# r9y9/deepvoice3_pytorch

Measured on AMD Instinct MI355X. Metric: mel-frames/sec/node (train step, deepvoice3_ljspeech), higher is better.
Workload: dtype f16x3

## Files before the change

### deepvoice3_pytorch_amd/csrc/api.hip

```cpp
#include "common.h"
#include <atomic>
#include <mutex>
#include <vector>
#include <string.h>

static thread_local char g_err[512] = "";

void dv3_set_error(const char* fmt, ...) {
  va_list ap;
  va_start(ap, fmt);
  vsnprintf(g_err, sizeof(g_err), fmt, ap);
  va_end(ap);
}

int g_dv3_last_conv = 0, g_dv3_last_wgrad = 0;

__device__ uint32_t g_dv3_range_events;
uint32_t* dv3_range_ctr() {
  static uint32_t* ptr = nullptr;
  static std::once_flag once;
  std::call_once(once, [] {
    void* p = nullptr;
    if (hipGetSymbolAddress(&p, HIP_SYMBOL(g_dv3_range_events)) == hipSuccess) ptr = (uint32_t*)p;
  });
// ... 50 lines not shown
  return DV3_OK;
}
extern "C" int dv3_graph_side_end(void* side_stream, void** exec_out, int32_t* n_nodes_out) {
  DV3_REQUIRE(side_stream && exec_out, "graph_side_end: null argument");
  hipGraph_t graph = nullptr;
  hipError_t e = hipStreamEndCapture((hipStream_t)side_stream, &graph);
  if (e != hipSuccess || !graph) {
    dv3_set_error("graph_side_end: hipStreamEndCapture: %s", hipGetErrorString(e));
    return DV3_ELAUNCH;
  }
  size_t n = 0;
  (void)hipGraphGetNodes(graph, nullptr, &n);
  if (n_nodes_out) *n_nodes_out = (int32_t)n;
  *exec_out = nullptr;
  if (n == 0) {
    (void)hipGraphDestroy(graph);
    return DV3_OK;
  }
  hipGraphExec_t exec = nullptr;
  e = hipGraphInstantiate(&exec, graph, nullptr, nullptr, 0);
  (void)hipGraphDestroy(graph);
  if (e != hipSuccess) {
    dv3_set_error("graph_side_end: hipGraphInstantiate: %s", hipGetErrorString(e));
    return DV3_ELAUNCH;
  }
  *exec_out = (void*)exec;
  return DV3_OK;
}
namespace {
__global__ void flag_signal_kernel(unsigned long long* flag, unsigned long long* epoch, int j, int bump) {
  unsigned long long e = *epoch;
  if (bump) {
    e += 1;
    *epoch = e;
  }
  __hip_atomic_store(flag, e * 4096ull + (unsigned long long)j, __ATOMIC_RELEASE, __HIP_MEMORY_SCOPE_AGENT);
}
__global__ void flag_wait_kernel(const unsigned long long* flag, unsigned long long* epoch, int j, int bump, unsigned* err,
                                 long long timeout_ticks) {
  unsigned long long e = *epoch;
  if (bump) {
    e += 1;
    *epoch = e;
  }
  const unsigned long long want = e * 4096ull + (unsigned long long)j;
  const long long t0 = (long long)wall_clock64();
  while (__hip_atomic_load(flag, __ATOMIC_ACQUIRE, __HIP_MEMORY_SCOPE_AGENT) < want) {
    __builtin_amdgcn_s_sleep(16);
    if ((long long)wall_clock64() - t0 > timeout_ticks) {
      atomicAdd(err, 1u);
      break;
    }
  }
}
}
extern "C" int dv3_flag_signal(uint64_t* flag, uint64_t* epoch, int32_t j, int32_t bump, void* stream) {
  DV3_REQUIRE(flag && epoch && j > 0 && j < 4096, "flag_signal: bad arguments");
  hipLaunchKernelGGL(flag_signal_kernel, dim3(1), dim3(1), 0, (hipStream_t)stream, (unsigned long long*)flag,
                     (unsigned long long*)epoch, (int)j, (int)bump);
  return dv3_check_launch("flag_signal");
}
extern "C" int dv3_flag_wait(const uint64_t* flag, uint64_t* epoch, int32_t j, int32_t bump, uint32_t* err,
                             int32_t timeout_ms, void* stream) {
  DV3_REQUIRE(flag && epoch && err && j > 0 && j < 4096 && timeout_ms > 0, "flag_wait: bad arguments");
  hipLaunchKernelGGL(flag_wait_kernel, dim3(1), dim3(1), 0, (hipStream_t)stream, (const unsigned long long*)flag,
                     (unsigned long long*)epoch, (int)j, (int)bump, (unsigned*)err, (long long)timeout_ms * 100000ll);
  return dv3_check_launch("flag_wait");
}
extern "C" int dv3_graph_launch(void* exec, void* stream) {
  DV3_REQUIRE(exec, "graph_launch: null graph");
  hipError_t e = hipGraphLaunch((hipGraphExec_t)exec, (hipStream_t)stream);
  if (e != hipSuccess) {
    dv3_set_error("graph_launch: %s", hipGetErrorString(e));
    return DV3_ELAUNCH;
  }
  return DV3_OK;
}
extern "C" int dv3_graph_destroy(void* exec) {
  if (exec) (void)hipGraphExecDestroy((hipGraphExec_t)exec);
  return DV3_OK;
}

int dv3_conv_census_count();
extern "C" int dv3_debug_get(int what) {
  if (what == 10) return g_dv3_last_conv;
  if (what == 40) return dv3_conv_census_count();
  if (what == 11) return g_dv3_last_wgrad;
  return 0;
}

extern int g_x3_pingpong, g_x3_rel2, g_x3_pp2, g_x3_prio, g_x3_wide, g_x3_pp2_sk_units, g_x3_j1_flat, g_x3_rel8;
extern int g_x3_ks, g_x3_ks_max_blocks, g_x3_ks_min_steps;
extern int g_pp2_ord_u, g_pp2_ord_m, g_pp2_sk, g_pp2_sk_overhead, g_pp2_sk_gain, g_pp2_fast_tail;
extern int g_planes_tile;
extern int g_c8pp_min_tiles, g_c8pp_rf, g_c8pp_nw4, g_c8pp_stagger, g_c8pp_stagger_mask;
extern int g_wgrad_tile, g_wgrad_prio, g_wgrad_taps2_default, g_wgrad_t2_window, g_wgrad_t2_il;
extern int g_wgrad_c8_pf2, g_wgrad_c8_il, g_wgrad_c8_tr;
extern int g_spk_prefetch;
extern int g_gate_c8_fast, g_gate_vec;
extern int g_loss_fast_log;
extern int g_wn_bwd_vec4;
int dv3_conv_census_set(int on);
extern "C" int dv3_debug_set(int what, int value) {
  if (what == 40) return dv3_conv_census_set(value);
  if (what == 29 || what == 31) {
    DV3_REQUIRE(value == 0 || value == 17 || value == 81, "debug_set(%d, %d): LOAD-phase order 0, 17 or 81", what, value);
    (what == 29 ? g_pp2_ord_u : g_pp2_ord_m) = value;
    return DV3_OK;
  }
  DV3_REQUIRE(what != 52 || (value >= 0 && value <= 4), "debug_set(52, %d): wgrad_c8 form 0..4", value);
  static const struct {
    int what;
    int* var;
  } kSwitches[] = {
      {2, &g_wgrad_tile},        {3, &g_x3_pingpong},         {4, &g_planes_tile},      {9, &g_x3_rel2},
      {12, &g_x3_pp2},           {14, &g_x3_prio},            {15, &g_wgrad_prio},      {17, &g_wgrad_taps2_default},
      {18, &g_x3_wide},          {19, &g_c8pp_min_tiles},     {20, &g_wgrad_c8_pf2},    {22, &g_pp2_sk},
      {23, &g_pp2_sk_overhead},  {24, &g_pp2_sk_gain},        {25, &g_x3_pp2_sk_units}, {27, &g_x3_j1_flat},
      {30, &g_c8pp_rf},          {34, &g_c8pp_nw4},           {35, &g_c8pp_stagger},    {36, &g_c8pp_stagger_mask},
      {42, &g_x3_rel8},          {44, &g_x3_ks},              {45, &g_x3_ks_max_blocks}, {46, &g_x3_ks_min_steps},
      {47, &g_wgrad_t2_window},  {48, &g_wgrad_t2_il},        {49, &g_wgrad_c8_il},     {50, &g_pp2_fast_tail},
      {51, &g_wn_bwd_vec4},      {52, &g_wgrad_c8_tr},        {54, &g_spk_prefetch},    {55, &g_gate_vec},
      {56, &g_gate_c8_fast},     {57, &g_loss_fast_log},
  };
  for (const auto& sw : kSwitches)
    if (sw.what == what) {
      *sw.var = value;
      return DV3_OK;
    }
  dv3_set_error("debug_set(%d, %d): no such switch", what, value);
  return DV3_EINVAL;
}

int dv3_decode_read_stamps(void* dst, int64_t bytes);
int dv3_conv_census_read(int what, void* dst, int64_t bytes);
extern "C" int dv3_debug_read(int what, void* dst, int64_t bytes) {
  if (what == 40 || what == 41) return dv3_conv_census_read(what, dst, bytes);
  if (what == 3 && dst) return dv3_decode_read_stamps(dst, bytes);
  dv3_set_error("debug_read(%d): no such buffer", what);
  return DV3_EINVAL;
}

extern "C" const char* dv3_last_error(void) { return g_err; }
extern "C" int dv3_abi_version(void) { return DV3_ABI_VERSION; }

extern "C" int dv3_device_info(int dev, char* name, int name_len, int* n_cu) {
  hipDeviceProp_t prop;
  hipError_t e = hipGetDeviceProperties(&prop, dev);
  if (e != hipSuccess) {
    dv3_set_error("hipGetDeviceProperties: %s", hipGetErrorString(e));
    return DV3_ELAUNCH;
  }
  if (name && name_len > 0) {
    strncpy(name, prop.gcnArchName, (size_t)name_len - 1);
    name[name_len - 1] = 0;
  }
  if (n_cu) *n_cu = prop.multiProcessorCount;
  return DV3_OK;
}

extern "C" int dv3_sizeof(const char* name) {
#define DV3_SZ(T) if (!strcmp(name, #T)) return (int)sizeof(T)
  DV3_SZ(dv3_conv_desc);
  DV3_SZ(dv3_wgrad_desc);
  DV3_SZ(dv3_wn_desc);
  DV3_SZ(dv3_wn_bwd_desc);
  DV3_SZ(dv3_gate_bwd_desc);
  DV3_SZ(dv3_softmax_desc);
  DV3_SZ(dv3_softmax_bwd_desc);
  DV3_SZ(dv3_spec_loss_desc);
  DV3_SZ(dv3_spec_items_desc);
  DV3_SZ(dv3_wn_multi_entry);
  DV3_SZ(dv3_conv_step_desc);
  DV3_SZ(dv3_attn_step_desc);
  DV3_SZ(dv3_decode_entry);
  DV3_SZ(dv3_decode_program);
  DV3_SZ(dv3_attn_fwd_desc);
  DV3_SZ(dv3_spk_layer);
  DV3_SZ(dv3_spk_desc);
  DV3_SZ(dv3_dropout_site);
#undef DV3_SZ
  return -1;
}
```

### deepvoice3_pytorch_amd/csrc/wgrad_gemm_bf16x3.hip

```cpp
#include "common.h"
#include <type_traits>

typedef __bf16 bf16x8 __attribute__((ext_vector_type(8)));
typedef __bf16 bf16x2 __attribute__((ext_vector_type(2)));
typedef float f32x2 __attribute__((ext_vector_type(2)));
typedef float f32x4u __attribute__((ext_vector_type(4), aligned(4)));

namespace {

struct WgradArgs {
  dv3_wgrad_desc d;
  int m_tiles, c_tiles;
  int prio = 0;
};

constexpr int BKT = 32;
constexpr int KB = 4;
constexpr int PAD = 2;

__device__ __forceinline__ void split8(const float (&v)[8], bf16x8& hi, bf16x8& lo) {
#pragma unroll
  for (int i = 0; i < 8; i += 2) {
    const f32x2 f = {v[i], v[i + 1]};
    const bf16x2 h = __builtin_convertvector(f, bf16x2);
// ... 350 lines not shown
    }
  };

  f32x16 acc[JT][2];
#pragma unroll
  for (int j = 0; j < JT; ++j)
#pragma unroll
    for (int a = 0; a < 2; ++a)
#pragma unroll
      for (int r = 0; r < 16; ++r) acc[j][a][r] = 0.f;

  auto mfma_step = [&](int cur) {
    const bf16x8* GsH = smem + cur * BUF;
    const bf16x8* GsL = GsH + KB * LDM;
#pragma unroll
    for (int ks = 0; ks < 2; ++ks) {
      const int k8 = 2 * ks + lhi;
      const int ai = k8 * LDM + wm * 64 + l31;
      const bf16x8 ah0 = GsH[ai], ah1 = GsH[ai + 32];
      bf16x8 al0 = ah0, al1 = ah1;
      if (TERMS == 3) { al0 = GsL[ai]; al1 = GsL[ai + 32]; }
#pragma unroll
      for (int j = 0; j < JT; ++j) {
        const bf16x8* XsH = GsH + GBUF + j * XTAP;
        const int xi = k8 * LDN + wc * 32 + l31;
        const bf16x8 bh = XsH[xi];
        if (TERMS == 1) {
          acc[j][0] = __builtin_amdgcn_mfma_f32_32x32x16_bf16(ah0, bh, acc[j][0], 0, 0, 0);
          acc[j][1] = __builtin_amdgcn_mfma_f32_32x32x16_bf16(ah1, bh, acc[j][1], 0, 0, 0);
          continue;
        }
        const bf16x8 bl = XsH[KB * LDN + xi];
        acc[j][0] = __builtin_amdgcn_mfma_f32_32x32x16_bf16(al0, bh, acc[j][0], 0, 0, 0);
        acc[j][1] = __builtin_amdgcn_mfma_f32_32x32x16_bf16(al1, bh, acc[j][1], 0, 0, 0);
        acc[j][0] = __builtin_amdgcn_mfma_f32_32x32x16_bf16(ah0, bl, acc[j][0], 0, 0, 0);
        acc[j][1] = __builtin_amdgcn_mfma_f32_32x32x16_bf16(ah1, bl, acc[j][1], 0, 0, 0);
        acc[j][0] = __builtin_amdgcn_mfma_f32_32x32x16_bf16(ah0, bh, acc[j][0], 0, 0, 0);
        acc[j][1] = __builtin_amdgcn_mfma_f32_32x32x16_bf16(ah1, bh, acc[j][1], 0, 0, 0);
      }
    }
  };
  using S0 = std::integral_constant<int, 0>;

  if (nsteps > 0) {
    load_step(0, S0{});
    write_step(0, S0{});
  }
  __syncthreads();
  const int prio = args.prio;
  for (int step = 0; step < nsteps; ++step) {
    if (prio == 1) __builtin_amdgcn_s_setprio(3);
    if (step + 1 < nsteps) load_step(step + 1, S0{});
    if (prio == 1) __builtin_amdgcn_s_setprio(0);
    if (prio == 2) __builtin_amdgcn_s_setprio(3);
    mfma_step(step & 1);
    if (prio == 2) __builtin_amdgcn_s_setprio(0);
    if (prio == 1) __builtin_amdgcn_s_setprio(3);
    if (step + 1 < nsteps) write_step((step + 1) & 1, S0{});
    if (prio == 1) __builtin_amdgcn_s_setprio(0);
    __syncthreads();
  }

  const float oscale = MASK ? p.drop_scale : 1.0f;
  const int c = c0 + wc * 32 + l31;
  if (c < Cin) {
#pragma unroll
    for (int j = 0; j < JT; ++j) {
      float* __restrict__ ob = p.out + (int64_t)s * p.out_ss + (int64_t)j * M * p.ldo;
#pragma unroll
      for (int mi = 0; mi < 2; ++mi)
#pragma unroll
        for (int r = 0; r < 16; ++r) {
          const int m = m0 + wm * 64 + mi * 32 + (r & 3) + 8 * (r >> 2) + 4 * lhi;
          if (m < M) ob[(int64_t)m * p.ldo + c] = acc[j][mi][r] * oscale;
        }
    }
  }
}

}

int g_wgrad_taps2_default = 1;
int dv3_wgrad_taps2_dispatch(const dv3_wgrad_desc* d, hipStream_t st);
int g_wgrad_taps_default = 1;
int g_wgrad_prio = 0;
int g_wgrad_tile = 0;

template <bool MASK, int TERMS>
static int launch_wgrad_taps_t(const WgradArgs& a, int64_t nb, hipStream_t st) {
  constexpr int LDM = 128 + PAD;
  constexpr size_t lds = (size_t)2 * (2 * KB * LDM + 3 * 2 * KB * LDM) * 16;
  static bool attr_set = false;
  if (!attr_set) {
    hipError_t e = hipFuncSetAttribute((const void*)wgrad_taps_kernel<MASK, TERMS>,
                                       hipFuncAttributeMaxDynamicSharedMemorySize, 160 * 1024);
    if (e != hipSuccess) {
      dv3_set_error("wgrad_taps: hipFuncSetAttribute: %s", hipGetErrorString(e));
      return DV3_ELAUNCH;
    }
    attr_set = true;
  }
  hipLaunchKernelGGL((wgrad_taps_kernel<MASK, TERMS>), dim3((unsigned)nb), dim3(512), lds, st, a);
  return dv3_check_launch("wgrad_taps");
}
static int launch_wgrad_taps(const WgradArgs& a, int64_t nb, hipStream_t st) {
  const dv3_wgrad_desc* d = &a.d;
  if (d->split_bf16 == 2)
    return d->xmask ? launch_wgrad_taps_t<true, 1>(a, nb, st) : launch_wgrad_taps_t<false, 1>(a, nb, st);
  return d->xmask ? launch_wgrad_taps_t<true, 3>(a, nb, st) : launch_wgrad_taps_t<false, 3>(a, nb, st);
}

template <int WM, int WN>
static int launch_wgrad_x3(const WgradArgs& a, int64_t nb, hipStream_t st) {
  const dv3_wgrad_desc* d = &a.d;
  dim3 grid((unsigned)nb), block(WM * WN * 64);
  if (d->split_bf16 == 2) {
    if (d->xmask) {
      hipLaunchKernelGGL((wgrad_gemm_bf16x3_kernel<WM, WN, true, 1>), grid, block, 0, st, a);
    } else {
      hipLaunchKernelGGL((wgrad_gemm_bf16x3_kernel<WM, WN, false, 1>), grid, block, 0, st, a);
    }
  } else if (d->xmask) {
    hipLaunchKernelGGL((wgrad_gemm_bf16x3_kernel<WM, WN, true, 3>), grid, block, 0, st, a);
  } else {
    hipLaunchKernelGGL((wgrad_gemm_bf16x3_kernel<WM, WN, false, 3>), grid, block, 0, st, a);
  }
  return dv3_check_launch("wgrad_gemm_bf16x3");
}

int dv3_wgrad_gemm_bf16x3_dispatch(const dv3_wgrad_desc* d, hipStream_t st) {
  if ((int64_t)d->B * d->g_bs + (int64_t)d->M * d->g_rs >= (1ll << 30) ||
      (int64_t)d->B * d->x_bs + (int64_t)d->Cin * d->x_rs >= (1ll << 30) ||
      (d->xmask && (int64_t)d->B * d->Cin * d->xmask_rs >= (1ll << 30)))
    return 1;
  WgradArgs a;
  a.d = *d;
  a.prio = g_wgrad_prio;
  if (d->J == 3 && d->k_split && d->split_bf16 != 2 && (g_wgrad_tile == 4 || (g_wgrad_tile == 0 && g_wgrad_taps2_default)) &&
      (int64_t)(d->B - 1) * d->g_bs + (int64_t)(d->M - 1) * d->g_rs + d->T >= 8 &&
      (int64_t)(d->B - 1) * d->x_bs + (int64_t)(d->Cin - 1) * d->x_rs + d->Tin >= 8)
    return dv3_wgrad_taps2_dispatch(d, st);
  if (d->J == 3 && d->k_split && (g_wgrad_tile == 3 || (g_wgrad_tile == 0 && g_wgrad_taps_default))) {
    a.m_tiles = dv3_cdiv(d->M, 128);
    a.c_tiles = dv3_cdiv(d->Cin, 128);
    const int64_t nb = (int64_t)a.m_tiles * a.c_tiles * d->n_slabs;
    DV3_REQUIRE(nb < (1ll << 31), "wgrad_gemm: grid too large");
    g_dv3_last_wgrad = (d->split_bf16 == 2 ? 4000 : 3000) + 30;
    return launch_wgrad_taps(a, nb, st);
  }
  const bool big = g_wgrad_tile == 2;
  const int bm = big ? 256 : 128;
  a.m_tiles = dv3_cdiv(d->M, bm);
  a.c_tiles = dv3_cdiv(d->Cin, 128);
  const int64_t nb = (int64_t)a.m_tiles * a.c_tiles * d->J * d->n_slabs;
  DV3_REQUIRE(nb < (1ll << 31), "wgrad_gemm: grid too large");
  g_dv3_last_wgrad = (d->split_bf16 == 2 ? 4000 : 3000) + (big ? 20 : 10);
  return big ? launch_wgrad_x3<4, 2>(a, nb, st) : launch_wgrad_x3<2, 2>(a, nb, st);
}
```

### deepvoice3_pytorch_amd/ops.py

```python
import contextlib
import ctypes
import functools
import math

import torch

from . import _lib
from ._lib import CONSTS, STRUCTS, _env_flag, _env_int, _env_str

EPI_LINEAR = CONSTS["DV3_EPI_LINEAR"]
EPI_RELU = CONSTS["DV3_EPI_RELU"]
EPI_SIGMOID = CONSTS["DV3_EPI_SIGMOID"]
EPI_GLU = CONSTS["DV3_EPI_GLU"]
EPI_HIGHWAY = CONSTS["DV3_EPI_HIGHWAY"]
EPI_DGRAD = CONSTS["DV3_EPI_DGRAD"]
EPI_SOFTSIGN = CONSTS["DV3_EPI_SOFTSIGN"]
STORE_BCT = CONSTS["DV3_STORE_BCT"]
STORE_INTERLEAVE2 = CONSTS["DV3_STORE_INTERLEAVE2"]

_conv_desc = STRUCTS["dv3_conv_desc"]
_wgrad_desc = STRUCTS["dv3_wgrad_desc"]
_wn_desc = STRUCTS["dv3_wn_desc"]
_wn_bwd_desc = STRUCTS["dv3_wn_bwd_desc"]
_gate_bwd_desc = STRUCTS["dv3_gate_bwd_desc"]
# ... 831 lines not shown
    return dv, dg, dbias


class WnBwdBatch(object):
    active = False
    group = CONSTS["DV3_WN_BWD_MULTI_MAX"]
    _q, _keep, _dv = [], [], set()

    @classmethod
    def add(cls, d, rows, keep):
        if d.dv in cls._dv:
            cls.flush()
        c = type(d)()
        ctypes.memmove(ctypes.byref(c), ctypes.byref(d), ctypes.sizeof(d))
        cls._q.append(c)
        cls._keep.append(keep)
        cls._dv.add(d.dv)
        if len(cls._q) >= cls.group:
            cls.flush()

    @classmethod
    def flush(cls):
        if not cls._q:
            return
        q, keep = cls._q, cls._keep
        cls._q, cls._keep, cls._dv = [], [], set()
        arr = (type(q[0]) * len(q))(*q)
        _lib.call("dv3_weight_norm_bwd_multi", ctypes.byref(arr), len(q), _stream())
        if SideStream.stream is not None:
            SideStream.retain(keep)

    @classmethod
    def discard(cls):
        cls._q, cls._keep, cls._dv = [], [], set()


def transpose(x, add=None, alpha=1.0):
    x = _c(_chk(x, "x"))
    B, R, C = x.shape
    y = torch.empty((B, C, R), dtype=torch.float32, device=x.device)
    _lib.call("dv3_transpose_f32", x.data_ptr(), y.data_ptr(), _ptr(add), B, R, C, float(alpha), _stream())
    return y


def axpby(a, b, alpha):
    a = _c(a)
    out = torch.empty_like(a)
    _lib.call("dv3_axpby_f32", a.data_ptr(), _ptr(_c(b) if b is not None else None), out.data_ptr(),
              a.numel(), float(alpha), _stream())
    return out


def _ksplit_count(total_steps, tiles, slots=512, min_steps=None, c8=False):
    if min_steps is None:
        min_steps = max(8, min(28, total_steps // 12)) if c8 else max(8, min(32, total_steps // 14))
    return _ksplit_count_c(total_steps, tiles, slots, min_steps)


@functools.lru_cache(maxsize=None)
def _ksplit_count_c(total_steps, tiles, slots, min_steps):
    s_max = max(1, total_steps // min_steps)
    if tiles >= slots:
        return 1
    best, best_eff = 1, 0.0
    for s in range(1, min(s_max, slots) + 1):
        blocks = tiles * s
        rounds = -(-blocks // slots)
        eff = blocks / float(rounds * slots)
        eff *= 1.0 - 0.008 * s
        if eff > best_eff:
            best, best_eff = s, eff
    return best


@functools.lru_cache(maxsize=None)
def _slab_count(B, tiles):
    want = max(1, (512 + tiles - 1) // tiles)
    s = min(B, want)
    while B % s:
        s -= 1
    return max(s, 1)


def wgrad_plan(B, Mg, Cin, Tg, Jd):
    tiles = ((Mg + 127) // 128) * ((Cin + 127) // 128) * Jd
    x3 = _gemm_mode != "f32" and not (Mg <= 64 and Cin <= 64)
    if x3 and Jd == 3:
        S = _ksplit_count(B * ((Tg + 31) // 32), tiles // 3, slots=256)
    elif x3:
        S = _ksplit_count(B * ((Tg + 31) // 32), tiles)
    else:
        S = _slab_count(B, tiles)
    return x3, S


class LayerCfg(object):
    __slots__ = ("k", "dil", "causal", "mode", "residual", "p", "training", "transposed", "site",
                 "pad_left", "t_out", "out_c8")

    def __init__(self, k=1, dil=1, causal=False, mode=EPI_LINEAR, residual=False, p=0.0,
                 training=False, transposed=False, site=None, pad_left=None, t_out=None, out_c8=None):
        self.k, self.dil, self.causal, self.mode = k, dil, causal, mode
        self.residual, self.p, self.training, self.transposed, self.site = residual, p, training, transposed, site
        self.pad_left, self.t_out = pad_left, t_out
        self.out_c8 = out_c8


def _pad_left(k, dil, causal):
    return (k - 1) * dil if causal else (k - 1) // 2 * dil


slab_rows_default = _env_flag("DV3_SLAB_ROWS", True)

grad_ready_hooks = []


class SideStream(object):
    stream = None
    main = None
    keep = []
    capturing = False
    split_capture = False
    split_on_fork = None
    release_every = 4
    _n = 0
    _events = []

    class _Section(object):

        def __enter__(self):
            _stream_override.handle = SideStream.stream.cuda_stream

        def __exit__(self, *exc):
            _stream_override.handle = None
            SideStream._release_point()
            return False

    forks_last = 0
    forks = 0

    @classmethod
    def fork(cls, *tensors):
        cls.forks += 1
        if cls.split_capture:
            if cls.split_on_fork is not None:
                cls.split_on_fork()
        else:
            _lib.call("dv3_stream_fork", cls.main.cuda_stream, cls.stream.cuda_stream)
        cls.keep.append([None, [tensors]])
        return cls._section

    @classmethod
    def retain(cls, *tensors):
        if cls.keep:
            cls.keep[-1][1].append(tensors)
        else:
            cls.keep.append([None, [tensors]])

    @classmethod
    def _release_point(cls):
        cls._n += 1
        if cls.capturing or cls.stream is None or cls._n % cls.release_every:
            return
        done = -1
        for i, (ev, _) in enumerate(cls.keep):
            if ev is not None:
                if not ev.query():
                    break
                done = i
        if done >= 0:
# ... 181 lines not shown
            ctx.has_bias = bias is not None
            ctx.save_for_backward(x, v, g, ab if gated else y)
            ctx.tok = ctx.prod = None
            split_modes = _gemm_mode in ("f16x3", "bf16x3")
            ctx.pair_ok = bool(gated and pair_words and split_modes and pk.bwd_s is not None and
                               split_only and ab.dtype == torch.float32 and (spk is None or spk.dim() == 2) and
                               not (M <= 64 and Cin <= 64))
            if fuse_gate_bwd and split_modes and pk.bwd_s is not None:
                if gated and ab.dtype == torch.float32 and spk is None and split_only and \
                        B * Cg * T <= fuse_gate_max_elems:
                    ctx.tok = _GateToken(ab, mode, int(cfg.residual), x if mode == EPI_HIGHWAY else None, Cg,
                                         pair=ctx.pair_ok)
                    y._dv3_tok = ctx.tok
                prod = getattr(x_in, "_dv3_tok", None) if (x_in is x and getattr(x_in, "_dv3_sole", False)) else None
                if prod is not None and prod.C == Cin and ctx.needs_input_grad[0] and Tout == T and \
                        (J_ - 1) * cfg.dil <= 64 and J_ <= 16:
                    ctx.prod = prod
        return y

    @staticmethod
    def backward(ctx, dy):
        cfg, pk = ctx.cfg, ctx.pk
        B, Cin, T, Tout, M, Cg, J, padL = ctx.dims
        x, v, g, saved = ctx.saved_tensors
        mode = cfg.mode
        gated = mode in (EPI_GLU, EPI_HIGHWAY)
        dy = _c(dy)
        rs2 = math.sqrt(0.5)
        dr = dr2 = dspk = None
        r_scale = 0.0
        n_part, g_pair, part_t = B, False, False
        if gated:
            glu_skip = mode == EPI_GLU and cfg.residual
            fused = getattr(dy, "_dv3_gate", None)
            if fused is not None and ctx.tok is not None and fused.tok is ctx.tok and dy._version == fused.version:
                dab, dres, part = fused.dab, fused.dres, fused.part
                n_part, g_pair, part_t = fused.n_part, fused.pair, True
                dy._dv3_gate = None
                gate_fuse_stats["fused"] += 1
            else:
                g_pair = ctx.pair_ok
                dab, dres, part = gate_bwd(dy, saved, x if mode == EPI_HIGHWAY else None, B=B, C=Cg, T=T,
                                           mode=mode, residual=int(cfg.residual), want_dres=(mode == EPI_HIGHWAY),
                                           pair=g_pair)
                gate_fuse_stats["standalone"] += 1
            if glu_skip:
                dres, r_scale = dy, rs2
            if ctx.spk_dim == 2:
                dspk = part[:, :Cg].contiguous()
            elif ctx.spk_dim == 3:
                dspk = dab[:, :Cg, :]
            gmat, Tg = dab, T
        elif cfg.transposed:
            O = pk.O
            _, _, part = gate_bwd(dy, None, None, B=B, C=O, T=2 * T, mode=EPI_LINEAR, want_dpre=False)
            gmat = torch.empty((B, 2 * O, T), dtype=torch.float32, device=dy.device)
            _lib.call("dv3_deinterleave2_f32", dy.data_ptr(), gmat.data_ptr(), B, O, T, _stream())
            dres, Tg = None, T
        else:
            dr, dr2, alpha = _strip_residual_scalings(ctx, dy, lambda d, a: axpby(d, None, a))
            need_y = mode in (EPI_RELU, EPI_SIGMOID, EPI_SOFTSIGN)
            if mode == EPI_LINEAR and alpha == 1.0:
                _, _, part = gate_bwd(dy, None, None, B=B, C=M, T=Tout, mode=EPI_LINEAR, want_dpre=False)
                gmat = dy
            else:
                gmat, _, part = gate_bwd(dy, saved if need_y else None, None, B=B, C=M, T=Tout, mode=mode,
                                         alpha=alpha)
            dres, Tg = None, Tout
        dx = dv = dg = dbias = None
        Mg = gmat.shape[1]
        Jd = 1 if cfg.transposed else J
        if ctx.needs_input_grad[0]:
            gate = None
            if ctx.prod is not None:
                t_ = ctx.prod
                gate = GateFuse(t_.ab, t_.mode, t_.residual, t_.x, pair=t_.pair)
            dx = conv_gemm(gmat, pk.bwd, pk.ldb, 0, B=B, Cin=Mg, Tin=Tg, M=Cin, Tout=T, J=Jd,
                           dil=cfg.dil, padL=(Jd - 1) * cfg.dil - padL, mode=EPI_DGRAD, r=dres, r_scale=r_scale,
                           ymask=ctx.bits, ymask_rs=ctx.bits_rs, drop_scale=ctx.dscale,
                           a_split=pk.bwd_s if _gemm_mode != "f32" else None, gate=gate, x_pair=g_pair)
            if gate is not None:
                dx._dv3_gate = _GateResult(ctx.prod, gate, dx._version)
        if ctx.needs_input_grad[1]:
            x3, S = wgrad_plan(B, Mg, Cin, Tg, Jd)
            slab_rows = slab_rows_default and S > 1

            def wgrad():
                return wgrad_gemm(gmat, x, B=B, M=Mg, Cin=Cin, T=Tg, Tin=T, J=Jd, dil=cfg.dil, padL=padL,
                                  n_slabs=S, xmask=ctx.bits, xmask_rs=ctx.bits_rs, drop_scale=ctx.dscale,
                                  split_bf16=x3, k_split=x3, rows_of_slabs=slab_rows, g_pair=g_pair), ()

            dv, dg, dbias = _wgrad_tail(ctx, wgrad, S, slab_rows, v, g, Cin, part, n_part=n_part, part_t=part_t,
                                        transposed=cfg.transposed, fork=(gmat, x, ctx.bits, part, dy))
        return dx, dv, dg, dbias, dspk, dr, dr2, None, None


fused_speaker_bias = _env_flag("DV3_FUSED_SPK", True)
_spk_layer_t, _spk_desc_t = STRUCTS["dv3_spk_layer"], STRUCTS["dv3_spk_desc"]
SPK_MAX_LAYERS = CONSTS["DV3_SPK_MAX_LAYERS"]


class SpeakerBiasBlockFn(torch.autograd.Function):

    @staticmethod
    def forward(ctx, e, holder, *params):
        L = len(params) // 3
        ctx.holder = holder
        B, E, T = e.shape
        if e.stride(2) != 1:
            e = e.contiguous()
        layers = (_spk_layer_t * L)()
        outs = []
        for l in range(L):
            v, g, b = params[3 * l:3 * l + 3]
            C = v.shape[0]
            if not v.is_contiguous() or v.numel() != C * E:
                raise RuntimeError("speaker_bias_block: (C, E) contiguous weights expected")
            o = torch.empty((B, C, T), dtype=torch.float32, device=e.device)
            y = layers[l]
            y.v, y.g, y.bias, y.out, y.C = v.data_ptr(), _ptr(g), _ptr(b), o.data_ptr(), C
            outs.append(o)
        d = _spk_desc_t()
        d.e, d.e_bs, d.e_rs, d.B, d.E, d.T, d.n_layers = e.data_ptr(), e.stride(0), e.stride(1), B, E, T, L
        _lib.call("dv3_speaker_bias_fwd_f32", ctypes.byref(d), layers, _stream())
        ctx.L = L
        ctx.save_for_backward(e, *params, *outs)
        return tuple(outs)

    @staticmethod
    def backward(ctx, *douts):
        L = ctx.L
        saved = ctx.saved_tensors
        e, params, outs = saved[0], saved[1:1 + 3 * L], saved[1 + 3 * L:]
        B, E, T = e.shape
        inplace = _grads_in_place([p for p in params if p is not None])
        layers = (_spk_layer_t * L)()
        keep, grads = [], []
        for l in range(L):
            v, g, b = params[3 * l:3 * l + 3]
            C = v.shape[0]
            y = layers[l]
            y.v, y.g, y.bias, y.out, y.C = v.data_ptr(), _ptr(g), _ptr(b), outs[l].data_ptr(), C
            c8g = ctx.holder.pop(l, None)
            if c8g is not None:
                do = douts[l]
                z = _spk_dummy.get(e.device)
                if do is not None and not (z is not None and do.data_ptr() == z.data_ptr() and all(st == 0 for st in do.stride())):
                    raise RuntimeError("speaker_bias_block: the bias of layer %d has a consumer besides its Conv1dGLU layer; "
                                       "its gradient can not be combined with the c8 hand-over (set DV3_FUSED_SPK=0)" % l)
                keep.append(c8g)
                y.dout, y.dout_c8p = c8g.data_ptr(), c8g.shape[1]
            else:
                do = douts[l]
                if do is None:
                    do = torch.zeros((B, C, T), dtype=torch.float32, device=e.device)
                elif do.stride(2) != 1 or do.dtype != torch.float32:
                    do = do.float().contiguous()
                keep.append(do)
                y.dout, y.dout_bs, y.dout_rs = do.data_ptr(), do.stride(0), do.stride(1)
            if inplace:
                gv, gg, gb = v.grad, (g.grad if g is not None else None), (b.grad if b is not None else None)
            else:
                gv = torch.zeros_like(v)
                gg = torch.zeros_like(g) if g is not None else None
                gb = torch.zeros_like(b) if b is not None else None
            y.dv, y.dg, y.dbias = gv.data_ptr(), _ptr(gg), _ptr(gb)
            grads += [gv, gg, gb]
# ... 809 lines not shown
```

Baseline: 3.800 million.

## Add dedicated split-bf16 wgrad kernel for 1-tap convolutions with larger M tiles

```diff
diff --git a/deepvoice3_pytorch_amd/csrc/api.hip b/deepvoice3_pytorch_amd/csrc/api.hip
--- a/deepvoice3_pytorch_amd/csrc/api.hip
+++ b/deepvoice3_pytorch_amd/csrc/api.hip
@@ -156,10 +156,12 @@
 }
 
 int dv3_conv_census_count();
+extern int g_wgrad_j1;
 extern "C" int dv3_debug_get(int what) {
   if (what == 10) return g_dv3_last_conv;
   if (what == 40) return dv3_conv_census_count();
   if (what == 11) return g_dv3_last_wgrad;
+  if (what == 58) return g_wgrad_j1;
   return 0;
 }
 
@@ -169,6 +171,7 @@
 extern int g_planes_tile;
 extern int g_c8pp_min_tiles, g_c8pp_rf, g_c8pp_nw4, g_c8pp_stagger, g_c8pp_stagger_mask;
 extern int g_wgrad_tile, g_wgrad_prio, g_wgrad_taps2_default, g_wgrad_t2_window, g_wgrad_t2_il;
+extern int g_wgrad_j1;
 extern int g_wgrad_c8_pf2, g_wgrad_c8_il, g_wgrad_c8_tr;
 extern int g_spk_prefetch;
 extern int g_gate_c8_fast, g_gate_vec;
@@ -183,6 +186,7 @@
     return DV3_OK;
   }
   DV3_REQUIRE(what != 52 || (value >= 0 && value <= 4), "debug_set(52, %d): wgrad_c8 form 0..4", value);
+  DV3_REQUIRE(what != 58 || (value >= 0 && value <= 3), "debug_set(58, %d): J = 1 wgrad form 0..3", value);
   static const struct {
     int what;
     int* var;
@@ -196,6 +200,7 @@
       {47, &g_wgrad_t2_window},  {48, &g_wgrad_t2_il},        {49, &g_wgrad_c8_il},     {50, &g_pp2_fast_tail},
       {51, &g_wn_bwd_vec4},      {52, &g_wgrad_c8_tr},        {54, &g_spk_prefetch},    {55, &g_gate_vec},
       {56, &g_gate_c8_fast},     {57, &g_loss_fast_log},
+      {58, &g_wgrad_j1},
   };
   for (const auto& sw : kSwitches)
     if (sw.what == what) {
diff --git a/deepvoice3_pytorch_amd/csrc/wgrad_gemm_bf16x3.hip b/deepvoice3_pytorch_amd/csrc/wgrad_gemm_bf16x3.hip
--- a/deepvoice3_pytorch_amd/csrc/wgrad_gemm_bf16x3.hip
+++ b/deepvoice3_pytorch_amd/csrc/wgrad_gemm_bf16x3.hip
@@ -456,6 +456,8 @@
 
 int g_wgrad_taps2_default = 1;
 int dv3_wgrad_taps2_dispatch(const dv3_wgrad_desc* d, hipStream_t st);
+bool dv3_wgrad_j1_serves(const dv3_wgrad_desc* d);
+int dv3_wgrad_j1_dispatch(const dv3_wgrad_desc* d, hipStream_t st);
 int g_wgrad_taps_default = 1;
 int g_wgrad_prio = 0;
 int g_wgrad_tile = 0;
@@ -510,6 +512,7 @@
   WgradArgs a;
   a.d = *d;
   a.prio = g_wgrad_prio;
+  if (g_wgrad_tile == 0 && dv3_wgrad_j1_serves(d)) return dv3_wgrad_j1_dispatch(d, st);
   if (d->J == 3 && d->k_split && d->split_bf16 != 2 && (g_wgrad_tile == 4 || (g_wgrad_tile == 0 && g_wgrad_taps2_default)) &&
       (int64_t)(d->B - 1) * d->g_bs + (int64_t)(d->M - 1) * d->g_rs + d->T >= 8 &&
       (int64_t)(d->B - 1) * d->x_bs + (int64_t)(d->Cin - 1) * d->x_rs + d->Tin >= 8)
diff --git a/deepvoice3_pytorch_amd/csrc/wgrad_j1.hip b/deepvoice3_pytorch_amd/csrc/wgrad_j1.hip
--- /dev/null
+++ b/deepvoice3_pytorch_amd/csrc/wgrad_j1.hip
@@ -0,0 +1,350 @@
+#include "common.h"
+#include <type_traits>
+
+typedef __bf16 bf16x8 __attribute__((ext_vector_type(8)));
+typedef __bf16 bf16x2 __attribute__((ext_vector_type(2)));
+typedef float f32x2 __attribute__((ext_vector_type(2)));
+typedef float f32x4u __attribute__((ext_vector_type(4), aligned(4)));
+
+namespace {
+
+struct WgradJ1Args {
+  dv3_wgrad_desc d;
+  int m_tiles, c_tiles;
+};
+
+constexpr int BKT = 32, KB = 4, PAD = 2;
+constexpr int BN = 128, NT = 512;
+constexpr int LDN = BN + PAD;
+
+__device__ __forceinline__ void wj1_split8(const float (&v)[8], bf16x8& hi, bf16x8& lo) {
+#pragma unroll
+  for (int i = 0; i < 8; i += 2) {
+    const f32x2 f = {v[i], v[i + 1]};
+    const bf16x2 h = __builtin_convertvector(f, bf16x2);
+    const f32x2 r = f - __builtin_convertvector(h, f32x2);
+    const bf16x2 l = __builtin_convertvector(r, bf16x2);
+    hi[i] = h[0]; hi[i + 1] = h[1];
+    lo[i] = l[0]; lo[i + 1] = l[1];
+  }
+}
+template <typename T>
+__device__ __forceinline__ T wj1_ldg(const void* base, uint32_t byte_off) {
+  return *reinterpret_cast<const T*>(reinterpret_cast<const char*>(base) + byte_off);
+}
+__device__ __forceinline__ uint32_t wj1_valid8(int t, int len) {
+  const int elo = max(0, -t), ehi = min(8, len - t);
+  return ehi > elo ? (((1u << ehi) - 1u) & ~((1u << elo) - 1u)) : 0u;
+}
+__device__ __forceinline__ void wj1_mask8(float (&v)[8], uint32_t m) {
+#pragma unroll
+  for (int e = 0; e < 8; ++e)
+    v[e] = __uint_as_float(__float_as_uint(v[e]) & (uint32_t)__builtin_amdgcn_sbfe((int)m, e, 1));
+}
+__device__ __forceinline__ void wj1_load8(const float* __restrict__ base, int off, int total, float (&v)[8]) {
+  const int offc = min(max(off, 0), total - 8);
+  const f32x4u a = wj1_ldg<f32x4u>(base, (uint32_t)offc * 4u);
+  const f32x4u b = wj1_ldg<f32x4u>(base, (uint32_t)offc * 4u + 16u);
+  v[0] = a[0]; v[1] = a[1]; v[2] = a[2]; v[3] = a[3];
+  v[4] = b[0]; v[5] = b[1]; v[6] = b[2]; v[7] = b[3];
+}
+__device__ __forceinline__ void wj1_realign(float (&v)[8], int sh) {
+  asm volatile("" : "+v"(sh));
+  float w[8];
+#pragma unroll
+  for (int e = 0; e < 8; ++e) {
+    float x = 0.f;
+#pragma unroll
+    for (int q = 0; q < 8; ++q) x = (e + sh == q) ? v[q] : x;
+    w[e] = x;
+  }
+#pragma unroll
+  for (int e = 0; e < 8; ++e) v[e] = w[e];
+}
+
+template <int NI, bool GP>
+__global__ __launch_bounds__(NT) void wgrad_j1_kernel(const WgradJ1Args args) {
+  static_assert(NI == 1 || NI == 2, "wave tile 64 x 32 or 64 x 64");
+  constexpr int WN = 4 / NI;
+  constexpr int BM = 64 * (8 / WN);
+  constexpr int LDM = BM + PAD;
+  constexpr int GU = BM * KB / NT;
+  constexpr int GBUF = 2 * KB * LDM, BUF = GBUF + 2 * KB * LDN;
+  constexpr int NM = 6 * NI;
+  constexpr int NST = 2 * (GU + 1);
+  constexpr int K1 = NI == 2 ? 6 : 8, K2 = NI == 2 ? 6 : 12;
+  const dv3_wgrad_desc& p = args.d;
+  extern __shared__ __attribute__((aligned(16))) unsigned char smem_raw_j1[];
+  bf16x8* const smem = reinterpret_cast<bf16x8*>(smem_raw_j1);
+
+  const int tid = threadIdx.x, lane = tid & 63;
+  const int wave = __builtin_amdgcn_readfirstlane(tid >> 6);
+  const int wm = wave / WN, wn = wave % WN;
+  const int l31 = lane & 31, lhi = lane >> 5;
+
+  int pid = dv3_xcd_remap(blockIdx.x, gridDim.x);
+  const int mt = pid % args.m_tiles; pid /= args.m_tiles;
+  const int ct = pid % args.c_tiles;
+  const int s = pid / args.c_tiles;
+  const int m0 = mt * BM, c0 = ct * BN;
+  const int T = p.T, Tin = p.Tin, M = p.M, Cin = p.Cin;
+  const int shift = -p.padL;
+
+  const int urow = tid >> 2, uk8 = tid & 3;
+  float rg[2][GU][8], rx[2][8];
+  const int n_tc = (T + BKT - 1) / BKT;
+  int nsteps, step0;
+  {
+    const int total = p.B * n_tc, q = (total + p.n_slabs - 1) / p.n_slabs;
+    step0 = s * q;
+    nsteps = max(0, min(q, total - step0));
+  }
+  const int g_total = (p.B - 1) * (int)p.g_bs + (M - 1) * (int)p.g_rs + T;
+  const int x_total = (p.B - 1) * (int)p.x_bs + (Cin - 1) * (int)p.x_rs + Tin;
+  int grow_off[GU];
+  bool grow_ok[GU];
+#pragma unroll
+  for (int u = 0; u < GU; ++u) {
+    const int m = m0 + urow + u * (NT / KB);
+    grow_ok[u] = m < M;
+    grow_off[u] = (m < M ? m : M - 1) * (int)p.g_rs + uk8 * 8;
+  }
+  const int xc = c0 + urow;
+  const bool xrow_ok = xc < Cin;
+  const int xrow_off = (xrow_ok ? xc : Cin - 1) * (int)p.x_rs + uk8 * 8 + shift;
+  uint32_t xrow_bits = xrow_ok ? 0xffu : 0u;
+  asm volatile("" : "+v"(xrow_bits));
+
+  auto step_coords = [&](int step, int& t0, int& gb, int& xb) __attribute__((always_inline)) {
+    const int gs = step0 + min(step, nsteps - 1);
+    const int b = gs / n_tc, tc = gs - b * n_tc;
+    t0 = tc * BKT;
+    gb = b * (int)p.g_bs + t0;
+    xb = b * (int)p.x_bs + t0;
+  };
+  auto load_step = [&](int step, auto set_c) __attribute__((always_inline)) {
+    constexpr int S = decltype(set_c)::value;
+    int t0, gb, xb;
+    step_coords(step, t0, gb, xb);
+#pragma unroll
+    for (int u = 0; u < GU; ++u) wj1_load8(p.g, gb + grow_off[u], g_total, rg[S][u]);
+    wj1_load8(p.x, xb + xrow_off, x_total, rx[S]);
+  };
+  auto fix_step = [&](int step, auto set_c) __attribute__((always_inline)) {
+    constexpr int S = decltype(set_c)::value;
+    int t0, gb, xb;
+    step_coords(step, t0, gb, xb);
+#pragma unroll
+    for (int u = 0; u < GU; ++u) {
+      const int off = gb + grow_off[u];
+      const int sh = off - min(max(off, 0), g_total - 8);
+      uint32_t vm = 0xffu;
+      if (t0 + BKT > T) vm = wj1_valid8(t0 + uk8 * 8, T);
+      if (!grow_ok[u]) vm = 0u;
+      if (__any(sh != 0)) wj1_realign(rg[S][u], sh);
+      if (__any(vm != 0xffu)) wj1_mask8(rg[S][u], vm);
+    }
+    {
+      const int off = xb + xrow_off;
+      const int sh = off - min(max(off, 0), x_total - 8);
+      if (__any(sh != 0)) wj1_realign(rx[S], sh);
+    }
+    return t0;
+  };
+  auto conv_g = [&](auto set_c, int u, bf16x8& hi, bf16x8& lo) __attribute__((always_inline)) {
+    constexpr int S = decltype(set_c)::value;
+    if constexpr (GP) {
+      uint32_t w[8];
+#pragma unroll
+      for (int e = 0; e < 8; ++e) w[e] = __float_as_uint(rg[S][u][e]);
+      dv3_pair_units(w, hi, lo);
+    } else wj1_split8(rg[S][u], hi, lo);
+  };
+  auto conv_x = [&](auto set_c, int t0, bf16x8& hi, bf16x8& lo) __attribute__((always_inline)) {
+    constexpr int S = decltype(set_c)::value;
+    const uint32_t xm = wj1_valid8(t0 + uk8 * 8 + shift, Tin) & xrow_bits;
+    float v[8];
+#pragma unroll
+    for (int e = 0; e < 8; ++e)
+      v[e] = __uint_as_float(__float_as_uint(rx[S][e]) & (uint32_t)__builtin_amdgcn_sbfe((int)xm, e, 1));
+    wj1_split8(v, hi, lo);
+  };
+  auto store_g = [&](int buf, int u, const bf16x8& hi, const bf16x8& lo) __attribute__((always_inline)) {
+    bf16x8* dst = smem + buf * BUF;
+    const int o = uk8 * LDM + urow + u * (NT / KB);
+    dst[o] = hi;
+    dst[KB * LDM + o] = lo;
+  };
+  auto store_x = [&](int buf, const bf16x8& hi, const bf16x8& lo) __attribute__((always_inline)) {
+    bf16x8* dx = smem + buf * BUF + GBUF;
+    const int o = uk8 * LDN + urow;
+    dx[o] = hi;
+    dx[KB * LDN + o] = lo;
+  };
+
+  f32x16 acc[2][NI];
+#pragma unroll
+  for (int a = 0; a < 2; ++a)
+#pragma unroll
+    for (int bq = 0; bq < NI; ++bq)
+#pragma unroll
+      for (int r = 0; r < 16; ++r) acc[a][bq][r] = 0.f;
+
+  auto mfma_ks = [&](int cur, auto ks_c) __attribute__((always_inline)) {
+    constexpr int ks = decltype(ks_c)::value;
+    const bf16x8* GsH = smem + cur * BUF;
+    const bf16x8* GsL = GsH + KB * LDM;
+    const bf16x8* XsH = GsH + GBUF;
+    const bf16x8* XsL = XsH + KB * LDN;
+    const int k8 = 2 * ks + lhi;
+    const int ai = k8 * LDM + wm * 64 + l31;
+    const int xi = k8 * LDN + wn * (32 * NI) + l31;
+    bf16x8 ah[2], al[2], bh[NI], bl[NI];
+#pragma unroll
+    for (int mi = 0; mi < 2; ++mi) { ah[mi] = GsH[ai + 32 * mi]; al[mi] = GsL[ai + 32 * mi]; }
+#pragma unroll
+    for (int ni = 0; ni < NI; ++ni) { bh[ni] = XsH[xi + 32 * ni]; bl[ni] = XsL[xi + 32 * ni]; }
+#pragma unroll
+    for (int mi = 0; mi < 2; ++mi)
+#pragma unroll
+      for (int ni = 0; ni < NI; ++ni)
+        acc[mi][ni] = __builtin_amdgcn_mfma_f32_32x32x16_bf16(al[mi], bh[ni], acc[mi][ni], 0, 0, 0);
+#pragma unroll
+    for (int mi = 0; mi < 2; ++mi)
+#pragma unroll
+      for (int ni = 0; ni < NI; ++ni)
+        acc[mi][ni] = __builtin_amdgcn_mfma_f32_32x32x16_bf16(ah[mi], bl[ni], acc[mi][ni], 0, 0, 0);
+#pragma unroll
+    for (int mi = 0; mi < 2; ++mi)
+#pragma unroll
+      for (int ni = 0; ni < NI; ++ni)
+        acc[mi][ni] = __builtin_amdgcn_mfma_f32_32x32x16_bf16(ah[mi], bh[ni], acc[mi][ni], 0, 0, 0);
+  };
+  using S0 = std::integral_constant<int, 0>;
+  using S1 = std::integral_constant<int, 1>;
+  using K0 = std::integral_constant<int, 0>;
+  using K1c = std::integral_constant<int, 1>;
+
+  if (nsteps > 0) {
+    load_step(0, S0{});
+    load_step(1, S1{});
+    {
+      const int t0 = fix_step(0, S0{});
+      bf16x8 hi, lo;
+#pragma unroll
+      for (int u = 0; u < GU; ++u) {
+        conv_g(S0{}, u, hi, lo);
+        store_g(0, u, hi, lo);
+      }
+      conv_x(S0{}, t0, hi, lo);
+      store_x(0, hi, lo);
+    }
+    load_step(2, S0{});
+    __syncthreads();
+
+    auto step = [&](int st, auto set_c) __attribute__((always_inline)) {
+      const int t0n = fix_step(st + 1, set_c);
+      bf16x8 ghi[GU], glo[GU], xhi, xlo;
+      __builtin_amdgcn_sched_barrier(0);
+      mfma_ks(st & 1, K0{});
+      conv_x(set_c, t0n, xhi, xlo);
+      if constexpr (GU == 2) conv_g(set_c, 0, ghi[0], glo[0]);
+      __builtin_amdgcn_sched_group_barrier(0x002, 8, 0);
+      __builtin_amdgcn_sched_group_barrier(0x100, 4 + 2 * NI, 0);
+#pragma unroll
+      for (int m = 0; m < NM; ++m) {
+        __builtin_amdgcn_sched_group_barrier(0x008, 1, 0);
+        __builtin_amdgcn_sched_group_barrier(0x002, K1, 0);
+      }
+      __builtin_amdgcn_sched_barrier(0);
+      mfma_ks(st & 1, K1c{});
+      conv_g(set_c, GU - 1, ghi[GU - 1], glo[GU - 1]);
+#pragma unroll
+      for (int u = 0; u < GU; ++u) store_g((st + 1) & 1, u, ghi[u], glo[u]);
+      store_x((st + 1) & 1, xhi, xlo);
+#pragma unroll
+      for (int m = 0; m < NM - NST; ++m) {
+        __builtin_amdgcn_sched_group_barrier(0x008, 1, 0);
+        __builtin_amdgcn_sched_group_barrier(0x002, K2, 0);
+      }
+#pragma unroll
+      for (int m = 0; m < NST; ++m) {
+        __builtin_amdgcn_sched_group_barrier(0x008, 1, 0);
+        __builtin_amdgcn_sched_group_barrier(0x200, 1, 0);
+      }
+      __builtin_amdgcn_sched_barrier(0);
+      load_step(st + 3, set_c);
+      __syncthreads();
+    };
+    int st = 0;
+    for (; st + 1 < nsteps; st += 2) {
+      step(st, S1{});
+      step(st + 1, S0{});
+    }
+    if (st < nsteps) step(st, S1{});
+  }
+
+  float* __restrict__ ob = p.out + (int64_t)s * p.out_ss;
+#pragma unroll
+  for (int mi = 0; mi < 2; ++mi)
+#pragma unroll
+    for (int ni = 0; ni < NI; ++ni) {
+      const int c = c0 + wn * (32 * NI) + ni * 32 + l31;
+      if (c >= Cin) continue;
+#pragma unroll
+      for (int r = 0; r < 16; ++r) {
+        const int m = m0 + wm * 64 + mi * 32 + (r & 3) + 8 * (r >> 2) + 4 * lhi;
+        if (m < M) ob[(int64_t)m * p.ldo + c] = acc[mi][ni][r];
+      }
+    }
+}
+
+template <int NI, bool GP>
+int launch_wgrad_j1(const WgradJ1Args& a, int64_t nb, hipStream_t st) {
+  constexpr int BM = NI == 2 ? 256 : 128;
+  constexpr size_t lds = (size_t)2 * (2 * KB * (BM + PAD) + 2 * KB * LDN) * 16;
+  static bool attr_set = false;
+  if (!attr_set) {
+    hipError_t e = hipFuncSetAttribute((const void*)wgrad_j1_kernel<NI, GP>, hipFuncAttributeMaxDynamicSharedMemorySize,
+                                       160 * 1024);
+    if (e != hipSuccess) {
+      dv3_set_error("wgrad_j1: hipFuncSetAttribute: %s", hipGetErrorString(e));
+      return DV3_ELAUNCH;
+    }
+    attr_set = true;
+  }
+  hipLaunchKernelGGL((wgrad_j1_kernel<NI, GP>), dim3((unsigned)nb), dim3(NT), lds, st, a);
+  return dv3_check_launch("wgrad_j1");
+}
+
+}
+
+int g_wgrad_j1 = 1;
+
+static bool dv3_wgrad_j1_big(const dv3_wgrad_desc* d) {
+  if (g_wgrad_j1 == 3 || d->M <= 128) return false;
+  if (g_wgrad_j1 == 2) return true;
+  return d->M > 256 && (int64_t)d->B * dv3_cdiv(d->T, BKT) >= 1024;
+}
+
+bool dv3_wgrad_j1_serves(const dv3_wgrad_desc* d) {
+  if (g_wgrad_j1 == 0) return false;
+  if (!(d->J == 1 && d->k_split && d->split_bf16 == 1 && !d->xmask)) return false;
+  if ((int64_t)(d->B - 1) * d->g_bs + (int64_t)(d->M - 1) * d->g_rs + d->T < 8 ||
+      (int64_t)(d->B - 1) * d->x_bs + (int64_t)(d->Cin - 1) * d->x_rs + d->Tin < 8)
+    return false;
+  return true;
+}
+
+int dv3_wgrad_j1_dispatch(const dv3_wgrad_desc* d, hipStream_t st) {
+  WgradJ1Args a;
+  a.d = *d;
+  const bool big = dv3_wgrad_j1_big(d);
+  a.m_tiles = dv3_cdiv(d->M, big ? 256 : 128);
+  a.c_tiles = dv3_cdiv(d->Cin, BN);
+  const int64_t nb = (int64_t)a.m_tiles * a.c_tiles * d->n_slabs;
+  DV3_REQUIRE(nb < (1ll << 31), "wgrad_gemm: grid too large");
+  g_dv3_last_wgrad = 3000 + (big ? 50 : 60) + (d->g_pair ? 1 : 0);
+  if (big) return d->g_pair ? launch_wgrad_j1<2, true>(a, nb, st) : launch_wgrad_j1<2, false>(a, nb, st);
+  return d->g_pair ? launch_wgrad_j1<1, true>(a, nb, st) : launch_wgrad_j1<1, false>(a, nb, st);
+}
diff --git a/deepvoice3_pytorch_amd/ops.py b/deepvoice3_pytorch_amd/ops.py
--- a/deepvoice3_pytorch_amd/ops.py
+++ b/deepvoice3_pytorch_amd/ops.py
@@ -937,10 +937,34 @@
     return max(s, 1)
 
 
-def wgrad_plan(B, Mg, Cin, Tg, Jd):
+WGRAD_J1_SWITCH = 58
+
+
+wgrad_j1_steps_cap = 16
+
+
+def wgrad_j1_form(B, Mg, Cin, Tg, Jd, masked=False):
+    if Jd != 1 or masked or _gemm_mode not in ("f16x3", "bf16x3"):
+        return 0
+    sw = _lib.lib().dv3_debug_get(WGRAD_J1_SWITCH)
+    if sw == 0:
+        return 0
+    if sw == 3 or Mg <= 128:
+        return 128
+    if sw == 2:
+        return 256
+    return 256 if (Mg > 256 and B * ((Tg + 31) // 32) >= 1024) else 128
+
+
+def wgrad_plan(B, Mg, Cin, Tg, Jd, masked=False):
     tiles = ((Mg + 127) // 128) * ((Cin + 127) // 128) * Jd
     x3 = _gemm_mode != "f32" and not (Mg <= 64 and Cin <= 64)
-    if x3 and Jd == 3:
+    bm = wgrad_j1_form(B, Mg, Cin, Tg, Jd, masked) if x3 else 0
+    if bm:
+        tiles = ((Mg + bm - 1) // bm) * ((Cin + 127) // 128)
+        total = B * ((Tg + 31) // 32)
+        S = _ksplit_count(total, tiles, slots=256, min_steps=max(8, min(wgrad_j1_steps_cap, total // 14)))
+    elif x3 and Jd == 3:
         S = _ksplit_count(B * ((Tg + 31) // 32), tiles // 3, slots=256)
     elif x3:
         S = _ksplit_count(B * ((Tg + 31) // 32), tiles)
@@ -1288,7 +1312,7 @@
             if gate is not None:
                 dx._dv3_gate = _GateResult(ctx.prod, gate, dx._version)
         if ctx.needs_input_grad[1]:
-            x3, S = wgrad_plan(B, Mg, Cin, Tg, Jd)
+            x3, S = wgrad_plan(B, Mg, Cin, Tg, Jd, masked=ctx.bits is not None)
             slab_rows = slab_rows_default and S > 1
 
             def wgrad():
```

Result: no change. 3.814 million (median of 4 runs) (+0.4%).
